# YifYang993/CR-NeRF-PyTorch

Measured on AMD Instinct MI355X. Metric: rays/sec (64+128 samples, 8-layer W=256 MLP), higher is better.
Workload: dtype f32

## Files before the change

cr-nerf-pytorch_amd/csrc/mlp_core16.h:

```cpp
#pragma once
#include <hip/hip_runtime.h>
#include "layout.h"
#include "sincos_pow2.h"
#include "mlp_core.h"

namespace crnerf {

#define CRNERF_MFMA16(a, b, c) __builtin_amdgcn_mfma_f32_16x16x4f32((a), (b), (c), 0, 0, 0)

constexpr int V16_WAVES = 8;
constexpr int V16_PIECES = STAGE_FRAGS / V16_WAVES;
constexpr int V16_AHEAD = 4;

constexpr int U_XYZ = XYZ_PAD / 16;
constexpr int U_HID = W_HIDDEN / 16;
constexpr int U_DIR = DIR_PAD / 16;
constexpr int U_HALF = 128 / 16;

constexpr int TRUNK_STAGES = OFF_FIN / STAGE_FRAGS;
static_assert(OFF_FIN % STAGE_FRAGS == 0, "the trunk must be whole stages");
template <bool TRUNK0>
struct WeightPipe16T {
  static constexpr bool trunk0 = TRUNK0;
  lds_char* lds;
  const char* base[2];
  const char* pf_ptr;
  int pf_left, pf_pass, passes0, passes;
  int stages_per_pass = STAGES_PER_PASS;
  uint32_t pf_slot, rd_slot, rd_addr, lane16, wave2k, lds_ring;
  int stagger;

  __device__ __forceinline__ void issue_piece(int i) {
    const uint32_t dst = lds_ring + pf_slot * STAGE_BYTES;
    if (i == 0) glds16(dst, pf_ptr, lane16, 0);
    else glds16(dst, pf_ptr, lane16, FRAG_BYTES);
    if (i == V16_PIECES - 1) {
      pf_slot = (pf_slot + 1 == RING_SLOTS) ? 0u : pf_slot + 1;
      pf_ptr += STAGE_BYTES;
      if (--pf_left == 0) {
        pf_left = stages_per_pass;
        pf_pass = (pf_pass + 1 == passes) ? 0 : pf_pass + 1;
        pf_ptr = (pf_pass < passes0) ? base[0] : base[1];
        if (TRUNK0 && pf_pass < passes0) pf_left = TRUNK_STAGES;
      }
    }
  }

  __device__ __forceinline__ void start(lds_char* lds_, const char* stream0, const char* stream1, int passes0_, int passes_,
                                        int lane, int wave) {
    static_assert(V16_PIECES == 2, "issue_piece hard-codes the two instruction offsets");
    lds = lds_;
    lane16 = (uint32_t)lane * 16u;
    wave2k = (uint32_t)wave * (V16_PIECES * FRAG_BYTES);
    lds_ring = (uint32_t)(uintptr_t)lds_ + LDS_RING + wave2k;
    stagger = (wave >> 2) & 1;
    base[0] = stream0 + wave2k;
    base[1] = stream1 + wave2k;
    passes0 = passes0_;
    passes = passes_;
    pf_pass = 0;
    pf_left = (TRUNK0 && passes0 > 0) ? TRUNK_STAGES : stages_per_pass;
    pf_ptr = (passes0 > 0) ? base[0] : base[1];
    pf_slot = 0;
    rd_slot = 0;
    rd_addr = LDS_RING + lane16;
#pragma unroll
    for (int s = 0; s < RING_SLOTS - 1; ++s)
#pragma unroll
      for (int i = 0; i < V16_PIECES; ++i) issue_piece(i);
    asm volatile("s_waitcnt vmcnt(%0)" ::"n"(V16_PIECES * (RING_SLOTS - 3)) : "memory");
    __builtin_amdgcn_s_barrier();
  }

  __device__ __forceinline__ uint32_t next_addr() const {
    const uint32_t n = (rd_slot + 1 == RING_SLOTS) ? 0u : rd_slot + 1;
    return LDS_RING + n * STAGE_BYTES + lane16;
  }

  __device__ __forceinline__ void advance() {
    asm volatile("s_waitcnt vmcnt(%0)" ::"n"(V16_PIECES * (RING_SLOTS - 4)) : "memory");
    __builtin_amdgcn_s_barrier();
    rd_slot = (rd_slot + 1 == RING_SLOTS) ? 0u : rd_slot + 1;
    rd_addr = LDS_RING + rd_slot * STAGE_BYTES + lane16;
  }

  __device__ __forceinline__ f32x4 read_slot(int s) const {
    const uint32_t a = (s < STAGE_FRAGS) ? rd_addr + s * FRAG_BYTES : next_addr() + (s - STAGE_FRAGS) * FRAG_BYTES;
    return *(const __attribute__((address_space(3))) f32x4*)(lds + a);
  }

  __device__ __forceinline__ void prime(f32x4 (&q)[V16_AHEAD]) const {
#pragma unroll
    for (int i = 0; i < V16_AHEAD; ++i) q[i] = read_slot(i);
  }
};
typedef WeightPipe16T<false> WeightPipe16;

template <int NT>
__device__ __forceinline__ void init_acc16(f32x4 (&acc)[NT], const lds_float* bias, int g) {
#pragma unroll
  for (int T = 0; T < NT; ++T) acc[T] = *(const __attribute__((address_space(3))) f32x4*)(bias + 16 * T + 4 * g);
}

struct NoDeferred {
  static constexpr int pieces = 0;
  __device__ __forceinline__ void piece(int) const {}
};
template <class SAVE, int ND>
struct DeferredActs {
  static constexpr int pieces = ND;
  const SAVE& save;
  float* row;
  const f32x4 (&a)[16];
  __device__ __forceinline__ void piece(int T) const { save.piece(row, T, a[T]); }
};

template <int NT, int NGA, int NGB, int NA, int NB, class DEF = NoDeferred, class PIPE>
__device__ __forceinline__ void mma_layer16(PIPE& p, const f32x4 (&srcA)[NA], const f32x4 (&srcB)[NB], f32x4 (&acc)[NT],
                                            f32x4 (&q)[V16_AHEAD], const DEF& def = DEF()) {
  static_assert(NGA <= NA && NGB <= NB, "source too small");
  constexpr int NF = (NGA + NGB) * NT;
  static_assert(NF % STAGE_FRAGS == 0 && NT % 2 == 0, "layer must be whole stages");
  constexpr int STEPS = NF / 2;
  constexpr int STRIDE = DEF::pieces > 0 ? (STEPS / DEF::pieces >= 4 ? 4 : (STEPS / DEF::pieces >= 2 ? 2 : 1)) : 1;
  static_assert(DEF::pieces == 0 || STRIDE * DEF::pieces <= STEPS, "not enough steps to carry the deferred stores");
#pragma unroll
  for (int u = 0; u < NGA + NGB; ++u) {
#pragma unroll
    for (int T = 0; T < NT; T += 2) {
      const int f = u * NT + T;
      const int s = f % STAGE_FRAGS;
      if (s % 4 == 0 && ((s >> 2) & 1) == p.stagger) p.issue_piece(s >> 3);
      const f32x4 a0 = q[f % V16_AHEAD], a1 = q[(f + 1) % V16_AHEAD];
      q[f % V16_AHEAD] = p.read_slot(s + V16_AHEAD);
      q[(f + 1) % V16_AHEAD] = p.read_slot(s + 1 + V16_AHEAD);
#pragma unroll
      for (int r = 0; r < 4; ++r) {
        const float b = (u < NGA) ? srcA[u < NGA ? u : 0][r] : srcB[u < NGA ? 0 : u - NGA][r];
        acc[T] = CRNERF_MFMA16(a0[r], b, acc[T]);
        acc[T + 1] = CRNERF_MFMA16(a1[r], b, acc[T + 1]);
      }
      if (s == STAGE_FRAGS - 2) p.advance();
      if (DEF::pieces > 0) {
        const int step = f / 2;
        if (step % STRIDE == 0 && step / STRIDE < DEF::pieces) def.piece(step / STRIDE);
      }
    }
  }
}

template <int NT, bool RELU, int NDST>
__device__ __forceinline__ void store_act16(const f32x4 (&acc)[NT], f32x4 (&act)[NDST]) {
#pragma unroll
  for (int T = 0; T < NT; ++T)
#pragma unroll
    for (int r = 0; r < 4; ++r) act[T][r] = RELU ? fmaxf(acc[T][r], 0.0f) : acc[T][r];
}

struct NoSave {
  template <int NT>
  __device__ __forceinline__ void operator()(int, const f32x4 (&)[NT]) const {}
  template <int NT>
  __device__ __forceinline__ float* begin(int, const f32x4 (&)[NT]) const { return nullptr; }
  __device__ __forceinline__ void piece(float*, int, const f32x4&) const {}
};

struct DirRegs {
  f32x4 v[2];
  __device__ __forceinline__ void get(f32x4 (&o)[2]) const { o[0] = v[0]; o[1] = v[1]; }
};
struct DirLds {
  const lds_float* p;
  __device__ __forceinline__ void get(f32x4 (&o)[2]) const {
    o[0] = *(const __attribute__((address_space(3))) f32x4*)(p);
    o[1] = *(const __attribute__((address_space(3))) f32x4*)(p + 4);
  }
};

template <class DIR, class SAVE = NoSave, class PIPE>
__device__ __forceinline__ void mlp_tile16(PIPE& p, int model, const f32x4 (&pe)[6], const DIR& dir,
                                           f32x4 (&feat)[4], float& sigma, int g, f32x4 (&q)[V16_AHEAD], PhaseTimer& tm,
                                           const SAVE& save = SAVE()) {
  const lds_float* C = (const lds_float*)(p.lds + (model ? LDS_CONST1 : LDS_CONST0));
  f32x4 act[16], acc[16];
  tm.tick(T_PROLOGUE);

  typedef DeferredActs<SAVE, 16> Def16;
  init_acc16<16>(acc, C + C_BIAS, g);
  mma_layer16<16, U_XYZ, 0>(p, pe, pe, acc, q);
  tm.tick(T_MMA);
  store_act16<16, true>(acc, act);
  float* row = save.begin(0, act);
#pragma unroll 1
  for (int l = 1; l < 4; ++l) {
    init_acc16<16>(acc, C + C_BIAS + l * W_HIDDEN, g);
    tm.tick(T_EPILOGUE);
    mma_layer16<16, U_HID, 0>(p, act, act, acc, q, Def16{save, row, act});
    tm.tick(T_MMA);
    store_act16<16, true>(acc, act);
    row = save.begin(l, act);
  }
  init_acc16<16>(acc, C + C_BIAS + 4 * W_HIDDEN, g);
  tm.tick(T_EPILOGUE);
  mma_layer16<16, U_XYZ, U_HID>(p, pe, act, acc, q, Def16{save, row, act});
  tm.tick(T_MMA);
  store_act16<16, true>(acc, act);
  row = save.begin(4, act);
#pragma unroll 1
  for (int l = 5; l < 8; ++l) {
    init_acc16<16>(acc, C + C_BIAS + l * W_HIDDEN, g);
    tm.tick(T_EPILOGUE);
    mma_layer16<16, U_HID, 0>(p, act, act, acc, q, Def16{save, row, act});
    tm.tick(T_MMA);
    store_act16<16, true>(acc, act);
    row = save.begin(l, act);
  }
  {
    float s0 = 0.0f, s1 = 0.0f;
#pragma unroll
    for (int T = 0; T < 16; T += 2) {
      const f32x4 w0 = *(const __attribute__((address_space(3))) f32x4*)(C + C_WSIG + 16 * T + 4 * g);
      const f32x4 w1 = *(const __attribute__((address_space(3))) f32x4*)(C + C_WSIG + 16 * (T + 1) + 4 * g);
#pragma unroll
      for (int r = 0; r < 4; ++r) {
        s0 = fmaf(w0[r], act[T][r], s0);
        s1 = fmaf(w1[r], act[T + 1][r], s1);
      }
    }
    float s = s0 + s1;
    s += __shfl_xor(s, 16);
    s += __shfl_xor(s, 32);
    sigma = softplus_ref(s + C[C_BSIG]);
  }
  tm.tick(T_SIGMA);
  if (PIPE::trunk0 && model == 0) {
#pragma unroll
    for (int T = 0; T < 4; ++T) feat[T] = f32x4{0, 0, 0, 0};
    return;
  }
  init_acc16<16>(acc, C + C_BFIN, g);
  mma_layer16<16, U_HID, 0>(p, act, act, acc, q, Def16{save, row, act});
  tm.tick(T_MMA);
  store_act16<16, false>(acc, act);
  row = save.begin(8, act);
  {
    f32x4 acc8[8], dv[2];
    dir.get(dv);
    init_acc16<8>(acc8, C + C_BDIR, g);
    tm.tick(T_EPILOGUE);
    mma_layer16<8, U_HID, U_DIR>(p, act, dv, acc8, q, Def16{save, row, act});
    tm.tick(T_MMA);
    store_act16<8, true>(acc8, act);
    row = save.begin(9, act);
  }
  {
    f32x4 acc4[4];
    init_acc16<4>(acc4, C + C_BRGB, g);
    tm.tick(T_EPILOGUE);
    mma_layer16<4, U_HALF, 0>(p, act, act, acc4, q, DeferredActs<SAVE, 8>{save, row, act});
    tm.tick(T_MMA);
#pragma unroll
    for (int T = 0; T < 4; ++T)
#pragma unroll
      for (int r = 0; r < 4; ++r) feat[T][r] = sigmoid_ref(acc4[T][r]);
  }
  tm.tick(T_EPILOGUE);
}

template <int F, int NV>
__device__ __forceinline__ void posenc_regs16(float x, float y, float z, int g, f32x4 (&out)[NV]) {
  const Rev2Pi rx = to_rev2pi(x), ry = to_rev2pi(y), rz = to_rev2pi(z);
#pragma unroll
  for (int v = 0; v < NV; ++v)
#pragma unroll
    for (int pr = 0; pr < 2; ++pr) {
      const int a_lo = 8 * v + pr;
      const int a = a_lo + 2 * g;
      float e0, e1;
      if (a_lo + 6 < 3 * F) {
        const int f = a / 3, d = a - 3 * f;
        const Rev2Pi val = {d == 0 ? rx.p : (d == 1 ? ry.p : rz.p), d == 0 ? rx.e : (d == 1 ? ry.e : rz.e)};
        float s, c;
        sincos_rev2pi(val, f, s, c);
        e0 = s; e1 = c;
      } else {
        const bool trig = a < 3 * F;
        const int ac = trig ? a : 0;
        const int f = ac / 3, d = ac - 3 * f;
        const Rev2Pi val = {d == 0 ? rx.p : (d == 1 ? ry.p : rz.p), d == 0 ? rx.e : (d == 1 ? ry.e : rz.e)};
        float s, c;
        sincos_rev2pi(val, f, s, c);
        e0 = trig ? s : (a == 3 * F ? x : (a == 3 * F + 1 ? z : 0.0f));
        e1 = trig ? c : (a == 3 * F ? y : 0.0f);
      }
      out[v][2 * pr + 0] = e0;
      out[v][2 * pr + 1] = e1;
    }
}

}
```

cr-nerf-pytorch_amd/csrc/mlp_forward16.hip:

```cpp
#include <hip/hip_runtime.h>
#include "kernels.h"
#include "mlp_core16.h"

namespace crnerf {

__global__ __launch_bounds__(512, 2) void mlp_forward16_kernel(const char* __restrict__ packed, const float* __restrict__ x,
                                                               float* __restrict__ out, int sigma_only, long P, int iters) {
  extern __shared__ __attribute__((aligned(16))) char smem[];
  lds_char* lds = (lds_char*)smem;
  const int lane = threadIdx.x & 63;
  const int wave = __builtin_amdgcn_readfirstlane(threadIdx.x >> 6);
  const int p = lane & 15, g = lane >> 4;

  load_consts(lds, packed, packed);
  WeightPipe16 pipe;
  pipe.start(lds, packed + CONST_BYTES, packed + CONST_BYTES, 1, 1, lane, wave);
  f32x4 q[V16_AHEAD];
  pipe.prime(q);
  PhaseTimer tm;
  tm.start(false);

#pragma unroll 1
  for (int it = 0; it < iters; ++it) {
    const long tile = ((long)it * gridDim.x + blockIdx.x) * V16_WAVES + wave;
    const long n = tile * 16 + p;
    const bool valid = n < P;
    const int xdim = sigma_only ? XYZ_DIM : IN_DIM;
    const float* row = x + (valid ? n : 0) * xdim;
    f32x4 pe[6], feat[4];
    DirRegs dreg;
    f32x4 (&dv)[2] = dreg.v;
#pragma unroll
    for (int v = 0; v < 6; ++v)
#pragma unroll
      for (int r = 0; r < 4; ++r) {
        const int c = posenc_slot_to_col16(16 * v + 4 * g + r, XYZ_FREQS);
        pe[v][r] = (valid && c >= 0) ? row[c < 0 ? 0 : c] : 0.0f;
      }
#pragma unroll
    for (int v = 0; v < 2; ++v)
#pragma unroll
      for (int r = 0; r < 4; ++r) {
        const int c = posenc_slot_to_col16(16 * v + 4 * g + r, DIR_FREQS);
        dv[v][r] = (valid && !sigma_only && c >= 0) ? row[XYZ_DIM + (c < 0 ? 0 : c)] : 0.0f;
      }
    float sigma;
    mlp_tile16(pipe, 0, pe, dreg, feat, sigma, g, q, tm);
    if (valid) {
      if (sigma_only) {
        if (g == 0) out[n] = sigma;
      } else {
        float* o = out + n * OUT_DIM;
#pragma unroll
        for (int T = 0; T < 4; ++T)
#pragma unroll
          for (int r = 0; r < 4; ++r) o[16 * T + 4 * g + r] = feat[T][r];
        if (g == 0) o[FEAT_DIM] = sigma;
      }
    }
  }
  asm volatile("s_waitcnt vmcnt(0)" ::: "memory");
}

int launch_mlp_forward16(const void* packed, const float* x, float* out, long P, int sigma_only, hipStream_t stream) {
  if (P <= 0) return 0;
  const long groups = (P + 127) / 128;
  const int cus = num_cus();
  const int grid = (int)(groups < cus ? groups : cus);
  const int iters = (int)((groups + grid - 1) / grid);
  const size_t shmem = LDS_SCRATCH;
  if (int rc = ensure_dynamic_lds((const void*)mlp_forward16_kernel, shmem, "mlp_forward16_kernel")) return rc;
  hipLaunchKernelGGL(mlp_forward16_kernel, dim3(grid), dim3(512), shmem, stream, (const char*)packed, x, out, sigma_only, P, iters);
  return check_launch("mlp_forward16_kernel");
}

}
```

cr-nerf-pytorch_amd/csrc/render_fused16.hip:

```cpp
#include <hip/hip_runtime.h>
#include "kernels.h"
#include "mlp_core16.h"
#include "mlp_train16.h"
#include "pair_ops.h"
#include "ray_ops.h"

namespace crnerf {

struct RenderParams16 {
  const char* packed0; const char* packed1;
  const float* rays; const float* view_dir; const float* z_coarse; const float* z_steps; const float* u; long u_stride;
  const float* noise_c; const float* noise_f; float noise_std; int use_disp;
  long R; int Nc, Ni, iters;
  unsigned int* sched;
  float* weights_c; float* feature_c; float* depth_c; float* weights_f; float* feature_f; float* depth_f; float* z_fine;
  unsigned long long rng_seed; long rng_ray_offset; int rng_flags; float perturb;
  float* z_coarse_out; float* noise_c_out; float* noise_f_out;
};

static __device__ unsigned int crnerf_sched16[SCHED_SLOTS][2];

struct NoHook {
  __device__ __forceinline__ NoSave saver(int, long, int, int, bool, int) const { return NoSave(); }
  __device__ __forceinline__ void raw(int, long, int, int, bool, int, const f32x4 (&)[4], float) const {}
};
struct TrainHook {
  float* acts[2];
  float* rawo[2];
  long R;
  __device__ __forceinline__ ActSaver saver(int pass, long r, int N, int n, bool ok, int g) const {
    return ActSaver{pass ? acts[1] : acts[0], R * N, r * N + n, ok, g};
  }
  __device__ __forceinline__ void raw(int pass, long r, int N, int n, bool ok, int g, const f32x4 (&feat)[4], float sigma) const {
    if (!ok) return;
    float* o = (pass ? rawo[1] : rawo[0]) + (r * N + n) * OUT_DIM;
#pragma unroll
    for (int T = 0; T < 4; ++T)
#pragma unroll
      for (int q = 0; q < 4; ++q) o[16 * T + 4 * g + q] = feat[T][q];
    if (g == 0) o[FEAT_DIM] = sigma;
  }
};

template <bool RNG, class HOOK, bool LEAN = false>
__device__ __forceinline__ void render_rays16_impl(const RenderParams16& a, const HOOK& hook) {
  extern __shared__ __attribute__((aligned(16))) char smem[];
  lds_char* lds = (lds_char*)smem;
  const int lane = threadIdx.x & 63;
  const int wave = __builtin_amdgcn_readfirstlane(threadIdx.x >> 6);
  const int p = lane & 15, g = lane >> 4;
  const int pair = wave >> 1, half = wave & 1;
  const int lane128 = half * 64 + lane;
  const int Nc = a.Nc, Ni = a.Ni, Nf = Nc + Ni;

  load_consts(lds, a.packed0, a.packed1);
  PairScratch scr;
  scr.bind(lds + LDS_SCRATCH + pair * PAIR_BYTES);
  lds_float* dirbuf = (lds_float*)(lds + LDS_SCRATCH + 4 * PAIR_BYTES) + wave * 32;

  const int steps_c = (Nc + 31) >> 5, steps_f = Ni > 0 ? (Nf + 31) >> 5 : 0;
  WeightPipe16T<LEAN> pipe;
  pipe.start(lds, a.packed0 + CONST_BYTES, a.packed1 + CONST_BYTES, steps_c, steps_c + steps_f, lane, wave);
  f32x4 q[V16_AHEAD];
  pipe.prime(q);
  PhaseTimer tm;
  tm.start(blockIdx.x == 0 && threadIdx.x == 0);

  __attribute__((address_space(3))) unsigned int* qslot =
      (__attribute__((address_space(3))) unsigned int*)(lds + LDS_SCRATCH + 4 * PAIR_BYTES + V16_WAVES * 32 * sizeof(float));
  const long quads = (a.R + 3) / 4;
  long quad = blockIdx.x;
#pragma unroll 1
  for (int it = 0; a.sched ? quad < quads : it < a.iters; ++it) {
    unsigned int nxt = 0;
    if (a.sched && threadIdx.x == 0) nxt = gridDim.x + atomicAdd(a.sched, 1u);
    const long rr = quad * 4 + pair;
    const bool ray_ok = rr < a.R;
    const long r = ray_ok ? rr : a.R - 1;
    const float* ray = a.rays + r * 8;
    const float ox = ray[0], oy = ray[1], oz = ray[2], dx = ray[3], dy = ray[4], dz = ray[5];
    const float near = ray[6], far = ray[7];
    {
      const float* vd = a.view_dir ? a.view_dir + r * 3 : ray + 3;
      f32x4 dv[2];
      posenc_regs16<DIR_FREQS, 2>(vd[0], vd[1], vd[2], g, dv);
      if (p == 0) {
        *(__attribute__((address_space(3))) f32x4*)(dirbuf + 8 * g) = dv[0];
        *(__attribute__((address_space(3))) f32x4*)(dirbuf + 8 * g + 4) = dv[1];
      }
    }
    const DirLds dirsrc{dirbuf + 8 * g};
    const RayRng rng{(uint32_t)(a.rng_seed & 0xffffffffu), (uint32_t)(a.rng_seed >> 32)};
    const long rng_ray = a.rng_ray_offset + r;
    for (int n = lane128; n < Nc; n += 128) {
      auto zlin = [&](int k) { return coarse_depth(near, far, a.z_steps ? a.z_steps[k] : linspace01(k, Nc), a.use_disp); };
      float zv;
      if (a.z_coarse) zv = a.z_coarse[r * Nc + n];
      else if (RNG && (a.rng_flags & 1)) {
        const float z0 = zlin(n);
        const float lower = n == 0 ? z0 : 0.5f * (zlin(n - 1) + z0);
        const float upper = n == Nc - 1 ? z0 : 0.5f * (z0 + zlin(n + 1));
        zv = lower + (upper - lower) * (a.perturb * rng.uniform(RNG_STREAM_JITTER, rng_ray, n));
      } else zv = zlin(n);
      scr.zc[n] = zv;
      if (RNG && a.z_coarse_out && ray_ok) a.z_coarse_out[r * Nc + n] = zv;
    }
    wg_barrier();

    const int npass = Ni > 0 ? 2 : 1;
#pragma unroll 1
    for (int pass = 0; pass < npass; ++pass) {
      const int N = pass ? Nf : Nc;
      const lds_float* zsrc = pass ? scr.zs : scr.zc;
      const float* noise_row = pass ? (a.noise_f ? a.noise_f + r * Nf : nullptr) : (a.noise_c ? a.noise_c + r * Nc : nullptr);
      float* weights_row = LEAN ? nullptr : (pass ? a.weights_f + r * Nf : a.weights_c + r * Nc);
      const bool compose = !LEAN || pass;
      double carry = 1.0;
      f32x4 facc[4];
#pragma unroll
      for (int T = 0; T < 4; ++T) facc[T] = f32x4{0, 0, 0, 0};
      float dacc = 0.0f;
      const int steps = (N + 31) >> 5;
#pragma unroll 1
      for (int k = 0; k < steps; ++k) {
        const int n = 32 * k + 16 * half + p;
        const bool valid = n < N;
        const int nc = valid ? n : N - 1;
        const float zn = zsrc[nc];
        const float znext = zsrc[nc + 1 < N ? nc + 1 : N - 1];
        const float x = ox + dx * zn, y = oy + dy * zn, z = oz + dz * zn;
        f32x4 pe[6], feat[4];
        posenc_regs16<XYZ_FREQS, 6>(x, y, z, g, pe);
        float sigma;
        mlp_tile16(pipe, pass, pe, dirsrc, feat, sigma, g, q, tm, hook.saver(pass, r, N, n, valid && ray_ok, g));
        hook.raw(pass, r, N, n, valid && ray_ok, g, feat, sigma);
        float noise = (noise_row && valid) ? noise_row[n] * a.noise_std : 0.0f;
        if (RNG && (a.rng_flags & 4) && valid) {
          const float draw = rng.normal(pass ? RNG_STREAM_NOISE_FINE : RNG_STREAM_NOISE_COARSE, rng_ray, n);
          noise = draw * a.noise_std;
          float* no = pass ? a.noise_f_out : a.noise_c_out;
          if (no && ray_ok && g == 0) no[r * N + n] = draw;
        }
        const float delta = (n == N - 1) ? 1e2f : znext - zn;
        const float alpha = valid ? 1.0f - expf(-delta * fmaxf(sigma + noise, 0.0f)) : 0.0f;
        double incl = (double)(1.0f - alpha);
#pragma unroll
        for (int d = 1; d < 16; d <<= 1) {
          const double o = shfl_up_f64(incl, d, 16);
          if (p >= d) incl *= o;
        }
        double excl = shfl_up_f64(incl, 1, 16);
        if (p == 0) excl = 1.0;
        const double tot = shfl_f64(incl, 15, 16);
        if (lane == 0) scr.xprod[half] = tot;
        wg_barrier();
        const double other = scr.xprod[half ^ 1];
        const double prod_a = half ? other : tot, prod_b = half ? tot : other;
        const float Tr = (float)(half ? carry * prod_a * excl : carry * excl);
        carry = carry * prod_a * prod_b;
        const float w = alpha * Tr;
        if (compose) {
#pragma unroll
          for (int T = 0; T < 4; ++T)
#pragma unroll
            for (int rr2 = 0; rr2 < 4; ++rr2) facc[T][rr2] += w * feat[T][rr2];
          dacc += w * zn;
        }
        if (valid && g == 0) {
          if (!LEAN && ray_ok) weights_row[n] = w;
          if (pass == 0) scr.wc[n] = w;
        }
        tm.tick(T_COMPOSITE);
      }
      {
#pragma unroll
        for (int d = 8; d >= 1; d >>= 1) if (compose) {
#pragma unroll
          for (int T = 0; T < 4; ++T)
#pragma unroll
            for (int rr2 = 0; rr2 < 4; ++rr2) facc[T][rr2] += __shfl_xor(facc[T][rr2], d);
          dacc += __shfl_xor(dacc, d);
        }
        if (compose && half == 1 && p == 0) {
#pragma unroll
          for (int T = 0; T < 4; ++T) *(__attribute__((address_space(3))) f32x4*)(scr.xfeat + 16 * T + 4 * g) = facc[T];
          if (g == 0) scr.xfeat[64] = dacc;
        }
      }
      wg_barrier();
      if (compose && half == 0 && p == 0 && ray_ok) {
        float* frow = (pass ? a.feature_f : a.feature_c) + r * FEAT_DIM;
#pragma unroll
        for (int T = 0; T < 4; ++T) {
          const f32x4 o = *(const __attribute__((address_space(3))) f32x4*)(scr.xfeat + 16 * T + 4 * g);
          *(f32x4*)(frow + 16 * T + 4 * g) = facc[T] + o;
        }
        if (g == 0) (pass ? a.depth_f : a.depth_c)[r] = dacc + scr.xfeat[64];
      }
      if (pass == 0 && Ni > 0) {
        sample_pdf_pair(scr, Nc, Ni, a.u ? a.u + r * a.u_stride : nullptr, lane, lane128, (RNG && (a.rng_flags & 2)) ? &rng : nullptr, rng_ray);
        wg_barrier();
        merge_sort_pair(scr, Nc, Ni, lane128);
        wg_barrier();
        if (a.z_fine && ray_ok)
          for (int n = lane128; n < Nf; n += 128) a.z_fine[r * Nf + n] = scr.zs[n];
      }
      tm.tick(T_RAYLEVEL);
    }
    if (a.sched && threadIdx.x == 0) *qslot = nxt;
    wg_barrier();
    quad = a.sched ? (long)__builtin_amdgcn_readfirstlane((int)*qslot) : quad + gridDim.x;
  }
  if (a.sched && threadIdx.x == 0 && atomicAdd(a.sched + 1, 1u) == gridDim.x - 1) {
    atomicExch(a.sched, 0u);
    atomicExch(a.sched + 1, 0u);
  }
  tm.flush();
  asm volatile("s_waitcnt vmcnt(0)" ::: "memory");
}

__global__ __launch_bounds__(512, 2) void render_rays16_kernel(RenderParams16 a) { render_rays16_impl<false>(a, NoHook{}); }
__global__ __launch_bounds__(512, 2) void render_rays16_rng_kernel(RenderParams16 a) { render_rays16_impl<true>(a, NoHook{}); }
__global__ __launch_bounds__(512, 2) void render_rays16_lean_kernel(RenderParams16 a) { render_rays16_impl<false, NoHook, true>(a, NoHook{}); }

__global__ __launch_bounds__(512, 2) void render_rays_train16_kernel(RenderParams16 a, TrainHook h) { render_rays16_impl<false>(a, h); }
__global__ __launch_bounds__(512, 2) void render_rays_train16_rng_kernel(RenderParams16 a, TrainHook h) { render_rays16_impl<true>(a, h); }

int launch_render_rays16(const RenderArgs& a, hipStream_t stream) {
  if (a.R <= 0) return 0;
  if (a.Nc < 2 || a.Nc > MAX_NC) return set_error(-2, "render_rays: N_samples must be in [2, 256] for the fused kernel");
  if (a.Ni < 0 || a.Ni > MAX_NI) return set_error(-2, "render_rays: N_importance must be in [0, 256] for the fused kernel");
  if (a.Ni > 0 && a.Nc < 3) return set_error(-2, "render_rays: hierarchical sampling needs N_samples >= 3");
  if (a.Ni > 0 && !a.packed_fine) return set_error(-3, "render_rays: N_importance > 0 but no fine model");
  RenderParams16 k;
  k.packed0 = (const char*)a.packed_coarse;
  k.packed1 = (const char*)(a.packed_fine ? a.packed_fine : a.packed_coarse);
  k.rays = a.rays; k.view_dir = a.view_dir; k.z_coarse = a.z_coarse; k.z_steps = a.z_steps; k.u = a.u; k.u_stride = a.u_stride;
  k.noise_c = a.noise_coarse; k.noise_f = a.noise_fine; k.noise_std = a.noise_std; k.use_disp = a.use_disp;
  k.R = a.R; k.Nc = a.Nc; k.Ni = a.Ni;
  k.weights_c = a.weights_coarse; k.feature_c = a.feature_coarse; k.depth_c = a.depth_coarse;
  k.weights_f = a.weights_fine; k.feature_f = a.feature_fine; k.depth_f = a.depth_fine; k.z_fine = a.z_fine;
  k.rng_seed = a.rng_seed; k.rng_ray_offset = a.rng_ray_offset; k.rng_flags = a.rng_flags; k.perturb = a.perturb;
  k.z_coarse_out = a.z_coarse_out; k.noise_c_out = a.noise_coarse_out; k.noise_f_out = a.noise_fine_out;
  const long quads = (a.R + 3) / 4;
  const int cus = num_cus();
  const int grid = (int)(quads < cus ? quads : cus);
  k.iters = (int)((quads + grid - 1) / grid);
  k.sched = k.iters > 1 ? sched_slot((const void*)crnerf_sched16) : nullptr;
  const size_t shmem = LDS_SCRATCH + 4 * PAIR_BYTES + V16_WAVES * 32 * sizeof(float) + 16;
  if (a.lean) {
    if (a.Ni < 1) return set_error(-2, "render_rays_lean: N_importance must be in [1, 256] (the coarse pass alone has nothing lean to return)");
    if (a.train_acts_coarse || a.rng_flags || a.z_coarse_out) return set_error(-3, "render_rays_lean: inference only, random draws come as tensors");
    if (int rc = ensure_dynamic_lds((const void*)render_rays16_lean_kernel, shmem, "render_rays16_lean_kernel")) return rc;
    hipLaunchKernelGGL(render_rays16_lean_kernel, dim3(grid), dim3(512), shmem, stream, k);
    return check_launch("render_rays16_lean_kernel");
  }
  if (a.train_acts_coarse) {
    if (a.Ni > 0 && (!a.train_acts_fine || !a.train_raw_fine)) return set_error(-1, "render_rays_train: fine buffers are NULL");
    if (!a.train_raw_coarse) return set_error(-1, "render_rays_train: raw_coarse is NULL");
    TrainHook h{{(float*)a.train_acts_coarse, (float*)a.train_acts_fine}, {a.train_raw_coarse, a.train_raw_fine}, a.R};
    if (int rc = zero_acts_range(a.train_acts_coarse, a.R * a.Nc, stream)) return rc;
    if (a.Ni > 0)
      if (int rc = zero_acts_range(a.train_acts_fine, a.R * (a.Nc + a.Ni), stream)) return rc;
    const bool rngk = a.rng_flags != 0 || a.z_coarse_out;
    const void* fn = rngk ? (const void*)render_rays_train16_rng_kernel : (const void*)render_rays_train16_kernel;
    if (int rc = ensure_dynamic_lds(fn, shmem, "render_rays_train16_kernel")) return rc;
    if (rngk) hipLaunchKernelGGL(render_rays_train16_rng_kernel, dim3(grid), dim3(512), shmem, stream, k, h);
    else hipLaunchKernelGGL(render_rays_train16_kernel, dim3(grid), dim3(512), shmem, stream, k, h);
    return check_launch("render_rays_train16_kernel");
  }
  const bool rngk = a.rng_flags != 0 || a.z_coarse_out;
  const void* fn = rngk ? (const void*)render_rays16_rng_kernel : (const void*)render_rays16_kernel;
  if (int rc = ensure_dynamic_lds(fn, shmem, "render_rays16_kernel")) return rc;
  if (rngk) hipLaunchKernelGGL(render_rays16_rng_kernel, dim3(grid), dim3(512), shmem, stream, k);
  else hipLaunchKernelGGL(render_rays16_kernel, dim3(grid), dim3(512), shmem, stream, k);
  return check_launch("render_rays16_kernel");
}

#ifdef CRNERF_TIMING
extern "C" int crnerf_debug_read_timing16(unsigned long long* host_out) {
  return (int)hipMemcpyFromSymbol(host_out, HIP_SYMBOL(crnerf_timing), sizeof(unsigned long long) * T_COUNT);
}
#endif

}
```

Measured before the change: 444,500.

## Stagger weight-ring barrier so half the waves rendezvous several steps earlier

The weight-streaming ring used to make all eight waves wait at one barrier after the last fragment pair of each stage. With a default lag of 6, waves 4..7 now hit their barrier six steps earlier with a tighter vmcnt, and their refill pieces move behind that barrier. Waves 0..3 issue their pieces at fixed early steps and keep the original end-of-stage wait. The goal is to reduce barrier stall and spread out global-to-LDS issue in the inference and render paths (training hooks keep lag 0). Static asserts check slot reuse, but the new ordering could race or leave waves idle if the reasoning is off.

```diff
diff --git a/cr-nerf-pytorch_amd/csrc/mlp_core16.h b/cr-nerf-pytorch_amd/csrc/mlp_core16.h
--- a/cr-nerf-pytorch_amd/csrc/mlp_core16.h
+++ b/cr-nerf-pytorch_amd/csrc/mlp_core16.h
@@ -12,6 +12,13 @@
 constexpr int V16_PIECES = STAGE_FRAGS / V16_WAVES;
 constexpr int V16_AHEAD = 4;
 
+#ifndef CRNERF_CORE16_LAG
+#define CRNERF_CORE16_LAG 6
+#endif
+#ifndef CRNERF_CORE16_PRIO
+#define CRNERF_CORE16_PRIO 0
+#endif
+
 constexpr int U_XYZ = XYZ_PAD / 16;
 constexpr int U_HID = W_HIDDEN / 16;
 constexpr int U_DIR = DIR_PAD / 16;
@@ -19,9 +26,25 @@
 
 constexpr int TRUNK_STAGES = OFF_FIN / STAGE_FRAGS;
 static_assert(OFF_FIN % STAGE_FRAGS == 0, "the trunk must be whole stages");
-template <bool TRUNK0>
+template <bool TRUNK0, int LAG = 0, bool PRIO = false>
 struct WeightPipe16T {
   static constexpr bool trunk0 = TRUNK0;
+  static constexpr int SYNC_S = STAGE_FRAGS - 2;
+  static constexpr int LATE_S = SYNC_S - LAG;
+  static constexpr int EARLY_P0 = 4, EARLY_P1 = 10;
+  static constexpr int LATE_P0 = LATE_S, LATE_P1 = LATE_S + 2;
+  static constexpr int SYNC_VMCNT = V16_PIECES * (RING_SLOTS - 4);
+  static constexpr int LATE_VMCNT = V16_PIECES * (RING_SLOTS - 5);
+  static_assert(LAG >= 0 && LAG % 2 == 0, "the barrier sits between fragment-pair steps");
+  static_assert(V16_WAVES == 8 && V16_PIECES * (V16_WAVES / 2) == STAGE_FRAGS / 2, "refill: waves 0..3 own fragments 0..7, waves 4..7 own 8..15");
+  static_assert(LATE_S >= STAGE_FRAGS / 2, "refill: behind b_(c-1) the early half rewrites fragments 0..7 of slot(c-1); the late half must have consumed them");
+  static_assert(LAG == 0 || (LATE_P0 >= LATE_S && LATE_P1 > LATE_P0 && LATE_P1 <= SYNC_S), "refill: the late half's pieces of stage c come behind its own b_c, inside stage c");
+  static_assert(EARLY_P0 >= 0 && EARLY_P1 > EARLY_P0 && EARLY_P1 <= SYNC_S, "certification: both early pieces of a stage are issued in front of its barrier");
+  static_assert(SYNC_VMCNT == 2 * V16_PIECES && LATE_VMCNT == V16_PIECES,
+                "certification: in flight at b_c are stage c + 4 and what the wave has issued of stage c + 5 (early: all, late: none); stage c + 3 has landed");
+  static_assert(LAG == 0 || ((LATE_P0 + LAG + 2) % STAGE_FRAGS != EARLY_P0 && (LATE_P0 + LAG + 2) % STAGE_FRAGS != EARLY_P1 &&
+                             (LATE_P1 + LAG + 2) % STAGE_FRAGS != EARLY_P0 && (LATE_P1 + LAG + 2) % STAGE_FRAGS != EARLY_P1),
+                "the partners' ~66-cycle piece issues must not coincide");
   lds_char* lds;
   const char* base[2];
   const char* pf_ptr;
@@ -54,6 +77,7 @@
     wave2k = (uint32_t)wave * (V16_PIECES * FRAG_BYTES);
     lds_ring = (uint32_t)(uintptr_t)lds_ + LDS_RING + wave2k;
     stagger = (wave >> 2) & 1;
+    if (PRIO && stagger) __builtin_amdgcn_s_setprio(1);
     base[0] = stream0 + wave2k;
     base[1] = stream1 + wave2k;
     passes0 = passes0_;
@@ -77,11 +101,41 @@
     return LDS_RING + n * STAGE_BYTES + lane16;
   }
 
-  __device__ __forceinline__ void advance() {
-    asm volatile("s_waitcnt vmcnt(%0)" ::"n"(V16_PIECES * (RING_SLOTS - 4)) : "memory");
+  __device__ __forceinline__ void rendezvous() {
+    asm volatile("s_waitcnt vmcnt(%0)" ::"n"(SYNC_VMCNT) : "memory");
     __builtin_amdgcn_s_barrier();
+  }
+  __device__ __forceinline__ void rendezvous_late() {
+    asm volatile("s_waitcnt vmcnt(%0)" ::"n"(LATE_VMCNT) : "memory");
+    __builtin_amdgcn_s_barrier();
+  }
+  __device__ __forceinline__ void bump() {
     rd_slot = (rd_slot + 1 == RING_SLOTS) ? 0u : rd_slot + 1;
     rd_addr = LDS_RING + rd_slot * STAGE_BYTES + lane16;
+  }
+  __device__ __forceinline__ void advance() {
+    rendezvous();
+    bump();
+  }
+  __device__ __forceinline__ void before_step(int s) {
+    if (LAG == 0) {
+      if (s % 4 == 0 && ((s >> 2) & 1) == stagger) issue_piece(s >> 3);
+    } else if (stagger) {
+      if (s == LATE_S) rendezvous_late();
+      if (s == LATE_P0) issue_piece(0);
+      if (s == LATE_P1) issue_piece(1);
+    } else {
+      if (s == EARLY_P0) issue_piece(0);
+      if (s == EARLY_P1) issue_piece(1);
+    }
+  }
+  __device__ __forceinline__ void after_step(int s) {
+    if (s != SYNC_S) return;
+    if (LAG == 0) advance();
+    else {
+      if (!stagger) rendezvous();
+      bump();
+    }
   }
 
   __device__ __forceinline__ f32x4 read_slot(int s) const {
@@ -95,6 +149,7 @@
   }
 };
 typedef WeightPipe16T<false> WeightPipe16;
+typedef WeightPipe16T<false, CRNERF_CORE16_LAG, CRNERF_CORE16_PRIO != 0> WeightPipe16Infer;
 
 template <int NT>
 __device__ __forceinline__ void init_acc16(f32x4 (&acc)[NT], const lds_float* bias, int g) {
@@ -130,7 +185,7 @@
     for (int T = 0; T < NT; T += 2) {
       const int f = u * NT + T;
       const int s = f % STAGE_FRAGS;
-      if (s % 4 == 0 && ((s >> 2) & 1) == p.stagger) p.issue_piece(s >> 3);
+      p.before_step(s);
       const f32x4 a0 = q[f % V16_AHEAD], a1 = q[(f + 1) % V16_AHEAD];
       q[f % V16_AHEAD] = p.read_slot(s + V16_AHEAD);
       q[(f + 1) % V16_AHEAD] = p.read_slot(s + 1 + V16_AHEAD);
@@ -140,7 +195,7 @@
         acc[T] = CRNERF_MFMA16(a0[r], b, acc[T]);
         acc[T + 1] = CRNERF_MFMA16(a1[r], b, acc[T + 1]);
       }
-      if (s == STAGE_FRAGS - 2) p.advance();
+      p.after_step(s);
       if (DEF::pieces > 0) {
         const int step = f / 2;
         if (step % STRIDE == 0 && step / STRIDE < DEF::pieces) def.piece(step / STRIDE);
diff --git a/cr-nerf-pytorch_amd/csrc/mlp_forward16.hip b/cr-nerf-pytorch_amd/csrc/mlp_forward16.hip
--- a/cr-nerf-pytorch_amd/csrc/mlp_forward16.hip
+++ b/cr-nerf-pytorch_amd/csrc/mlp_forward16.hip
@@ -13,7 +13,7 @@
   const int p = lane & 15, g = lane >> 4;
 
   load_consts(lds, packed, packed);
-  WeightPipe16 pipe;
+  WeightPipe16Infer pipe;
   pipe.start(lds, packed + CONST_BYTES, packed + CONST_BYTES, 1, 1, lane, wave);
   f32x4 q[V16_AHEAD];
   pipe.prime(q);
diff --git a/cr-nerf-pytorch_amd/csrc/render_fused16.hip b/cr-nerf-pytorch_amd/csrc/render_fused16.hip
--- a/cr-nerf-pytorch_amd/csrc/render_fused16.hip
+++ b/cr-nerf-pytorch_amd/csrc/render_fused16.hip
@@ -21,10 +21,12 @@
 static __device__ unsigned int crnerf_sched16[SCHED_SLOTS][2];
 
 struct NoHook {
+  static constexpr bool train = false;
   __device__ __forceinline__ NoSave saver(int, long, int, int, bool, int) const { return NoSave(); }
   __device__ __forceinline__ void raw(int, long, int, int, bool, int, const f32x4 (&)[4], float) const {}
 };
 struct TrainHook {
+  static constexpr bool train = true;
   float* acts[2];
   float* rawo[2];
   long R;
@@ -59,7 +61,7 @@
   lds_float* dirbuf = (lds_float*)(lds + LDS_SCRATCH + 4 * PAIR_BYTES) + wave * 32;
 
   const int steps_c = (Nc + 31) >> 5, steps_f = Ni > 0 ? (Nf + 31) >> 5 : 0;
-  WeightPipe16T<LEAN> pipe;
+  WeightPipe16T<LEAN, HOOK::train ? 0 : CRNERF_CORE16_LAG, !HOOK::train && CRNERF_CORE16_PRIO != 0> pipe;
   pipe.start(lds, a.packed0 + CONST_BYTES, a.packed1 + CONST_BYTES, steps_c, steps_c + steps_f, lane, wave);
   f32x4 q[V16_AHEAD];
   pipe.prime(q);
```

Measured after the change: 452,500, median of 6. 1.02x the previous value.
